# tenstack/batch-scheduler

Measured on NVIDIA H100. Metric: pod_x_node_fit_evals_per_sec, higher is better.
Workload: dtype int64

## Files before the change

### batch-scheduler_b200/csrc/fit.cuh

```cuda
#pragma once
#include "common.cuh"

namespace bsk {

__device__ __forceinline__ uint32_t smem_u32(const void* p) {
  return (uint32_t)__cvta_generic_to_shared(p);
}
__device__ __forceinline__ void mbar_init(uint64_t* bar, uint32_t count) {
  asm volatile("mbarrier.init.shared::cta.b64 [%0], %1;" ::"r"(smem_u32(bar)), "r"(count));
}
__device__ __forceinline__ void mbar_expect_tx(uint64_t* bar, uint32_t bytes) {
  asm volatile("mbarrier.arrive.expect_tx.shared::cta.b64 _, [%0], %1;" ::"r"(smem_u32(bar)), "r"(bytes)
               : "memory");
}
__device__ __forceinline__ void mbar_arrive(uint64_t* bar) {
  asm volatile("mbarrier.arrive.shared::cta.b64 _, [%0];" ::"r"(smem_u32(bar)) : "memory");
}
__device__ __forceinline__ void mbar_wait(uint64_t* bar, uint32_t parity) {
  asm volatile(
      "{\n"
      ".reg .pred p;\n"
      "WAIT_%=:\n"
      "mbarrier.try_wait.parity.shared::cta.b64 p, [%0], %1;\n"
      "@p bra DONE_%=;\n"
// ... 63 lines not shown
  uint32_t* fit_bitmap;
  int64_t* score;
  uint64_t left_w_pitch, left_n_pitch;
  uint64_t score_pitch;
  uint32_t bitmap_pitch;
  uint32_t P, N, Npad, W;
  uint32_t n_full, tail_split;
  unsigned long long* best_packed;
  int32_t* topk_node;
  int64_t* topk_score;
  uint32_t topk_k;
};

template <bool NARROW> struct BestT { using type = int64_t; };
template <> struct BestT<true> { using type = int32_t; };

enum { FIT_OUT_NONE = 0, FIT_OUT_BITMAP = 1, FIT_OUT_SCORE = 2, FIT_OUT_TOPK = 3 };

template <typename S>
__device__ __forceinline__ S topk_insert(S* __restrict__ ls_p, int32_t* __restrict__ ln_p, uint32_t K, uint32_t cb,
                                         S s, int32_t n0 , uint32_t lane) {
  S ls = ls_p[lane];
  int32_t ln = ln_p[lane];
#pragma unroll 1
  do {
    const uint32_t src = __ffs(cb) - 1;
    cb &= cb - 1;
    const S cs = __shfl_sync(0xffffffffu, s, src);
    const int32_t cn = n0 + (int32_t)src;
    const uint32_t pos = __popc(__ballot_sync(0xffffffffu, ls > cs || (ls == cs && ln < cn)));
    if (pos < K) {
      const S us = __shfl_up_sync(0xffffffffu, ls, 1);
      const int32_t un = __shfl_up_sync(0xffffffffu, ln, 1);
      if (lane == pos) { ls = cs; ln = cn; }
      else if (lane > pos) { ls = us; ln = un; }
    }
  } while (cb);
  ls_p[lane] = ls;
  ln_p[lane] = ln;
  return __shfl_sync(0xffffffffu, ls, K - 1);
}

template <int LW, int LN, int LS, int OUT, int RN>
__device__ __forceinline__ void fit_tile(const FitArgs& a, const int64_t* __restrict__ tlw,
                                         const int32_t* __restrict__ tln,
                                         const int64_t (&rqw)[PODS_PER_WARP][LW > 0 ? LW : 1],
                                         const int32_t (&rqn)[PODS_PER_WARP][LN + LS > 0 ? LN + LS : 1],
                                         const ColBits (&colbits)[PODS_PER_WARP], int R0, uint32_t slab ,
                                         uint32_t* s_words, uint32_t wbase , uint32_t node_base, uint32_t lane,
                                         typename BestT<(LN > 0)>::type (&best_s)[PODS_PER_WARP],
                                         int32_t (&best_n)[PODS_PER_WARP], int32_t (&kb)[PODS_PER_WARP],
                                         uint32_t (&cnt)[PODS_PER_WARP],
                                         typename BestT<(LN > 0)>::type* tks, int32_t* tkn ,
                                         typename BestT<(LN > 0)>::type (&thr)[PODS_PER_WARP]) {
  constexpr bool SCORE = OUT == FIT_OUT_SCORE;
  constexpr bool TOPK = OUT == FIT_OUT_TOPK;
  constexpr bool WORDS = OUT == FIT_OUT_BITMAP || SCORE;
  using S = typename BestT<(LN > 0)>::type;
  static_assert(!SCORE || RN == 1, "a staging slab holds one matrix row");
  const int64_t* tpw = tlw + lane;
  const int32_t* tpn = tln + lane;
  int32_t node = (int32_t)(node_base + lane);
  uint32_t wp = smem_u32(s_words) + wbase * 4;
  uint32_t sp = slab + lane * 8;
  int32_t jrem = TILE_WORDS - 1;
#pragma unroll 1
  for (int jb = 0; jb < TILE_WORDS; jb += 4) {
#pragma unroll
    for (int jj = 0; jj < 4; ++jj) {
      int64_t lfw[LW > 0 ? LW : 1];
      int32_t lfn[LN + LS > 0 ? LN + LS : 1];
#pragma unroll
      for (int d = 0; d < LW; ++d) lfw[d] = tpw[d * NODE_TILE + jj * 32];
#pragma unroll
      for (int d = 0; d < LN + LS; ++d) lfn[d] = tpn[d * NODE_TILE + jj * 32];
#pragma unroll
      for (int i = 0; i < RN; ++i) {
        const int r = R0 + i;
        if (LN > 0) {
          int32_t t = lfn[0] - rqn[r][0];
#pragma unroll
          for (int d = 1; d < LN; ++d) t = min(t, lfn[d] - rqn[r][d]);
          uint32_t m32 = (uint32_t)t;
          int32_t sgn = t;
#pragma unroll
          for (int d = 0; d < LS; ++d) {
            const int32_t x = min(lfn[LN + d] - rqn[r][LN + d], (int32_t)a.lm.sclamp[d]);
            sgn |= x;
            m32 = min(m32, (uint32_t)x << a.lm.sshift[d]);
          }
#pragma unroll
          for (int d = 0; d < LW; ++d) {
            const int64_t w = lfw[d] - rqw[r][d];
            const int32_t whi = hi32(w);
            sgn |= whi;
            m32 = min(m32, whi != 0 ? 0xffffffffu : lo32(w));
          }
          const bool fit = (sgn >= 0) && ((colbits[r] >> (jb + jj)) & 1u);
          if (WORDS) sts_u32(wp + (r * 32 + jj) * 4, __ballot_sync(0xffffffffu, fit));
          else if (fit) ++cnt[r];
          if (TOPK && a.fit_bitmap) sts_u32(wp + (r * 32 + jj) * 4, __ballot_sync(0xffffffffu, fit));
          const int32_t key = (int32_t)(m32 << KEY_BITS) + (jrem - jj);
          if (!TOPK && fit) kb[r] = max(kb[r], key);
          if (SCORE) sts_v2u32(sp + jj * 32 * 8, fit ? m32 : 0u, fit ? 0u : 0x80000000u);
          if (TOPK) {
            const uint32_t cb = __ballot_sync(0xffffffffu, fit && (int32_t)m32 > thr[r]);
            if (cb) thr[r] = topk_insert<S>(tks + r * 32, tkn + r * 32, a.topk_k, cb, (int32_t)m32, node + jj * 32 - (int32_t)lane, lane);
          }
        } else {
          int64_t m = lfw[0] - rqw[r][0];
#pragma unroll
          for (int d = 1; d < LW; ++d) m = min64(m, lfw[d] - rqw[r][d]);
          const bool fit = (hi32(m) >= 0) && ((colbits[r] >> (jb + jj)) & 1u);
          if (WORDS) sts_u32(wp + (r * 32 + jj) * 4, __ballot_sync(0xffffffffu, fit));
          else if (fit) ++cnt[r];
          if (TOPK && a.fit_bitmap) sts_u32(wp + (r * 32 + jj) * 4, __ballot_sync(0xffffffffu, fit));
          if (!TOPK && fit && m > best_s[r]) { best_s[r] = m; best_n[r] = node + jj * 32; }
          if (SCORE) sts_u64(sp + jj * 32 * 8, fit ? (long long)m : (long long)INT64_MIN);
          if (TOPK) {
            const uint32_t cb = __ballot_sync(0xffffffffu, fit && m > thr[r]);
            if (cb) thr[r] = topk_insert<S>(tks + r * 32, tkn + r * 32, a.topk_k, cb, m, node + jj * 32 - (int32_t)lane, lane);
          }
        }
      }
    }
    tpw += 128;
    tpn += 128;
    node += 128;
    jrem -= 4;
    wp += 16;
    sp += 128 * 8;
  }
}

__host__ __device__ constexpr size_t fit_tile_bytes(int LW, int LN, int LS) {
  return (size_t)NODE_TILE * (8 * LW + 4 * (LN + LS));
}
__host__ __device__ constexpr size_t fit_slab_bytes() { return (size_t)NODE_TILE * 8; }
__host__ __device__ constexpr size_t fit_topk_bytes() { return (size_t)PODS_PER_CTA * BS_TOPK_MAX * 12; }
static_assert(BS_TOPK_MAX == 32, "a top-K list holds one entry per lane");
__host__ __device__ constexpr size_t fit_smem_front(int LW, int LN, int LS) {
  size_t b = FIT_STAGES * fit_tile_bytes(LW, LN, LS) + (size_t)PODS_PER_CTA * (8 * LW + 4 * (LN + LS));
  b = (b + 7) & ~(size_t)7;
  b += 2 * FIT_STAGES * sizeof(uint64_t) + (size_t)PODS_PER_CTA * 32 * sizeof(uint32_t);
  return (b + 127) & ~(size_t)127;
}
__host__ __device__ constexpr size_t fit_smem_total(int LW, int LN, int LS, int out) {
  return fit_smem_front(LW, LN, LS) + (out == FIT_OUT_SCORE  ? (size_t)FIT_WARPS * FIT_NB * fit_slab_bytes()
                                       : out == FIT_OUT_TOPK ? fit_topk_bytes()
                                                             : 0);
}
constexpr size_t FIT_SMEM_MAX = 227 * 1024;

template <int LW, int LN, int LS, int OUT>
__global__ void __launch_bounds__(FIT_THREADS, FIT_MIN_BLOCKS) gang_fit_kernel(FitArgs a) {
  constexpr bool SCORE = OUT == FIT_OUT_SCORE;
  constexpr bool TOPK = OUT == FIT_OUT_TOPK;
  constexpr bool WORDS = OUT == FIT_OUT_BITMAP || SCORE;
  extern __shared__ __align__(128) unsigned char smem_raw[];
  constexpr size_t STAGE_BYTES = fit_tile_bytes(LW, LN, LS);
  constexpr int LNS = LN + LS;
  unsigned char* s_tile = smem_raw;
  int64_t* s_req_w = reinterpret_cast<int64_t*>(smem_raw + FIT_STAGES * STAGE_BYTES);
  int32_t* s_req_n = reinterpret_cast<int32_t*>(s_req_w + PODS_PER_CTA * LW);
  uint64_t* s_bar = reinterpret_cast<uint64_t*>(
      (reinterpret_cast<uintptr_t>(s_req_n + PODS_PER_CTA * LNS) + 7) & ~(uintptr_t)7);
  uint64_t* s_full = s_bar;
  uint64_t* s_empty = s_bar + FIT_STAGES;
  uint32_t* s_words_all = reinterpret_cast<uint32_t*>(s_bar + 2 * FIT_STAGES);

  const uint32_t tid = threadIdx.x, lane = tid & 31, wid = tid >> 5;
  uint32_t* s_words = s_words_all + wid * PODS_PER_WARP * 32;
  uint32_t unit = blockIdx.x, piece = 0, npieces = 1;
  if (blockIdx.x >= a.n_full) {
    const uint32_t tl = blockIdx.x - a.n_full;
    unit = a.n_full + tl / a.tail_split;
    piece = tl % a.tail_split;
    npieces = a.tail_split;
  }
  const uint32_t pod0 = unit * PODS_PER_CTA;
  const uint32_t wpod0 = pod0 + wid * PODS_PER_WARP;
  const uint32_t n_tiles = a.Npad / NODE_TILE;
  const uint32_t n_lines = (n_tiles + TILES_PER_LINE - 1) / TILES_PER_LINE;
  const uint32_t tile_lo = min(n_tiles, (n_lines * piece / npieces) * TILES_PER_LINE);
  const uint32_t tile_hi = min(n_tiles, (n_lines * (piece + 1) / npieces) * TILES_PER_LINE);

  if (tid == 0) {
    for (int st = 0; st < FIT_STAGES; ++st) {
      mbar_init(&s_full[st], 1);
      mbar_init(&s_empty[st], FIT_WARPS);
    }
    asm volatile("fence.mbarrier_init.release.cluster;" ::: "memory");
  }
  for (uint32_t i = tid; i < PODS_PER_CTA * (LW + LNS); i += FIT_THREADS) {
    const uint32_t pl = i / (LW + LNS), k = i % (LW + LNS);
    const uint32_t p = pod0 + pl;
    const bool is_w = k < (uint32_t)LW;
    const uint32_t kn = k - LW;
    const uint32_t d = is_w ? a.lm.wide[k] : (kn < (uint32_t)LN ? a.lm.narrow[kn] : a.lm.scaled[kn - LN]);
    int64_t v = 0;
    bool present = true;
    if (p < a.P) {
      present = d < 4 || ((a.req_present[p] >> d) & 1u);
      v = present ? a.req[(size_t)d * a.P + p] : 0;
    }
    if (is_w) s_req_w[pl * LW + k] = present ? v : UNCHECKED_REQ;
    else if (kn < (uint32_t)LN) s_req_n[pl * LNS + kn] = present ? (int32_t)v : UNCHECKED_REQ32;
    else s_req_n[pl * LNS + kn] = present ? (int32_t)(v >> a.lm.sunit[kn - LN]) : UNCHECKED_REQS;
  }
  __syncthreads();
  auto issue = [&](uint32_t tile, uint32_t stage) {
    mbar_expect_tx(&s_full[stage], (uint32_t)STAGE_BYTES);
    unsigned char* dst = s_tile + stage * STAGE_BYTES;
    const unsigned char* src_w = reinterpret_cast<const unsigned char*>(a.left_w) + (uint64_t)tile * (NODE_TILE * 8);
    const unsigned char* src_n = reinterpret_cast<const unsigned char*>(a.left_n) + (uint64_t)tile * (NODE_TILE * 4);
#pragma unroll
    for (int d = 0; d < LW; ++d)
      tma_bulk_g2s(dst + (size_t)d * NODE_TILE * 8, src_w + (uint64_t)d * a.left_w_pitch, NODE_TILE * 8,
                   &s_full[stage]);
#pragma unroll
    for (int d = 0; d < LNS; ++d)
      tma_bulk_g2s(dst + (size_t)LW * NODE_TILE * 8 + (size_t)d * NODE_TILE * 4,
                   src_n + (uint64_t)d * a.left_n_pitch, NODE_TILE * 4, &s_full[stage]);
  };
  if (wid == FIT_WARPS) {
    if (lane == 0) {
      if constexpr (SCORE) {
        const uint32_t range = tile_hi - tile_lo;
        for (uint32_t i = 0; i < PODS_PER_WARP * range; ++i) {
          const uint32_t st = i % FIT_STAGES, use = i / FIT_STAGES;
          if (use > 0) mbar_wait(&s_empty[st], (use - 1) & 1);
          issue(tile_lo + i % range, st);
        }
      } else {
        for (uint32_t tile = tile_lo; tile < tile_hi; ++tile) {
          const uint32_t st = (tile - tile_lo) % FIT_STAGES, use = (tile - tile_lo) / FIT_STAGES;
          if (use > 0) mbar_wait(&s_empty[st], (use - 1) & 1);
          issue(tile, st);
        }
      }
    }
    return;
  }

  const bool want_bitmap = a.fit_bitmap != nullptr;
  uint32_t cnt[PODS_PER_WARP];
  typename BestT<(LN > 0)>::type best_s[PODS_PER_WARP];
  int32_t best_n[PODS_PER_WARP];
  int32_t kb[PODS_PER_WARP], kthr[PODS_PER_WARP];
  typename BestT<(LN > 0)>::type thr[PODS_PER_WARP];
  int64_t rqw[PODS_PER_WARP][LW > 0 ? LW : 1];
  int32_t rqn[PODS_PER_WARP][LNS > 0 ? LNS : 1];
  uint32_t coff[PODS_PER_WARP];
  auto load_req = [&](int r) {
#pragma unroll
    for (int d = 0; d < LW; ++d) rqw[r][d] = s_req_w[(wid * PODS_PER_WARP + r) * LW + d];
#pragma unroll
    for (int d = 0; d < LNS; ++d) rqn[r][d] = s_req_n[(wid * PODS_PER_WARP + r) * LNS + d];
  };
  typename BestT<(LN > 0)>::type* tks =
      reinterpret_cast<typename BestT<(LN > 0)>::type*>(smem_raw + fit_smem_front(LW, LN, LS)) + wid * PODS_PER_WARP * 32;
  int32_t* tkn = reinterpret_cast<int32_t*>(smem_raw + fit_smem_front(LW, LN, LS) + (size_t)PODS_PER_CTA * 32 * 8) +
                 wid * PODS_PER_WARP * 32;
#pragma unroll
  for (int r = 0; r < PODS_PER_WARP; ++r) {
    cnt[r] = 0; best_n[r] = -1; kb[r] = -1; kthr[r] = 0; thr[r] = -1;
    if (TOPK) { tks[r * 32 + lane] = -1; tkn[r * 32 + lane] = -1; }
    best_s[r] = LN > 0 ? (typename BestT<(LN > 0)>::type)(-1) : (typename BestT<(LN > 0)>::type)INT64_MIN;
    const uint32_t p = wpod0 + r;
    coff[r] = (p < a.P ? a.fit_class[p] : 0u) * n_tiles * 32 + lane;
    if (!SCORE) load_req(r);
  }
  const uint32_t slab0 = smem_u32(smem_raw + fit_smem_front(LW, LN, LS)) + wid * (uint32_t)(FIT_NB * fit_slab_bytes());
  int64_t* srow = SCORE ? a.score + (size_t)wpod0 * a.score_pitch : nullptr;

  uint32_t stage = 0, phase = 0;
  constexpr int PASSES = SCORE ? PODS_PER_WARP : 1;
  uint32_t nseg = 0, nline = 0;
  ColBits colnext[PODS_PER_WARP];
#pragma unroll
  for (int pass = 0; pass < PASSES; ++pass) {
  if (SCORE) load_req(pass);
#pragma unroll
  for (int r = 0; r < PODS_PER_WARP; ++r)
    if (!SCORE || r == pass) colnext[r] = __ldg(a.classfit + coff[r] + min(tile_lo, n_tiles - 1) * 32);
  for (uint32_t tile = tile_lo; tile < tile_hi; ++tile) {
    ColBits colbits[PODS_PER_WARP];
    const uint32_t tnext = tile + 1 < tile_hi ? tile + 1 : tile;
#pragma unroll
    for (int r = 0; r < PODS_PER_WARP; ++r) {
      if (SCORE && r != pass) continue;
      colbits[r] = colnext[r];
      colnext[r] = __ldg(a.classfit + coff[r] + tnext * 32);
    }
    mbar_wait(&s_full[stage], phase);
    const int64_t* tlw = reinterpret_cast<const int64_t*>(s_tile + stage * STAGE_BYTES);
    const int32_t* tln = reinterpret_cast<const int32_t*>(s_tile + stage * STAGE_BYTES + (size_t)LW * NODE_TILE * 8);
    const uint32_t node_base = tile * NODE_TILE;
    const uint32_t wbase = (tile % TILES_PER_LINE) * TILE_WORDS;
    if constexpr (SCORE) {
      static_assert(PODS_PER_WARP >= FIT_NB, "a bitmap line's word row must be read before it is rewritten");
      const uint32_t wrow = nline % PODS_PER_WARP;
      const uint32_t slab = slab0 + (nseg % FIT_NB) * (uint32_t)fit_slab_bytes();
      if (nseg >= (uint32_t)FIT_NB) {
        if (lane == 0) bulk_wait_read<FIT_NB - 1>();
        __syncwarp();
      }
      fit_tile<LW, LN, LS, OUT, 1>(a, tlw, tln, rqw, rqn, colbits, pass, slab, s_words + ((int)wrow - pass) * 32, wbase,
                                   node_base, lane, best_s, best_n, kb, cnt, tks, tkn, thr);
      fence_async_smem();
      __syncwarp();
      if (lane == 0) {
        if (node_base < (uint32_t)a.score_pitch) {
          const uint32_t cols = min((uint32_t)NODE_TILE, (uint32_t)a.score_pitch - node_base);
          tma_bulk_s2g(srow + (size_t)pass * a.score_pitch + node_base, slab, cols * 8, l2_evict_first());
        }
        if (want_bitmap && ((tile + 1) % TILES_PER_LINE == 0 || tile + 1 == tile_hi))
          tma_bulk_s2g(a.fit_bitmap + (size_t)(wpod0 + pass) * a.bitmap_pitch + (tile / TILES_PER_LINE) * 32,
                       smem_u32(s_words + wrow * 32), (tile % TILES_PER_LINE + 1) * TILE_WORDS * 4, l2_evict_first());
        bulk_commit();
      }
      ++nseg;
    } else {
      fit_tile<LW, LN, LS, OUT, PODS_PER_WARP>(a, tlw, tln, rqw, rqn, colbits, 0, 0, s_words, wbase, node_base, lane,
                                               best_s, best_n, kb, cnt, tks, tkn, thr);
    }
    if (LN > 0 && !TOPK) {
#pragma unroll
      for (int r = 0; r < PODS_PER_WARP; ++r) {
        if (SCORE && r != pass) continue;
        if (kb[r] >= kthr[r]) {
          best_s[r] = kb[r] >> KEY_BITS;
          best_n[r] = (int32_t)(node_base + lane) + (TILE_WORDS - 1 - (kb[r] & (TILE_WORDS - 1))) * 32;
          kthr[r] = (best_s[r] + 1) << KEY_BITS;
        }
        kb[r] = -1;
      }
    }
    __syncwarp();
    if (lane == 0) mbar_arrive(&s_empty[stage]);
    if ((WORDS || (TOPK && want_bitmap)) && ((tile + 1) % TILES_PER_LINE == 0 || tile + 1 == tile_hi)) {
      const uint32_t line = tile / TILES_PER_LINE;
      const uint32_t valid = (tile % TILES_PER_LINE + 1) * TILE_WORDS;
      if constexpr (SCORE) {
        if (lane < valid) cnt[pass] += __popc(s_words[(nline % PODS_PER_WARP) * 32 + lane]);
        ++nline;
      } else if (lane < valid) {
#pragma unroll
        for (int r = 0; r < PODS_PER_WARP; ++r) {
          const uint32_t w = s_words[r * 32 + lane];
          if (WORDS) cnt[r] += __popc(w);
          if (want_bitmap) a.fit_bitmap[(size_t)(wpod0 + r) * a.bitmap_pitch + line * 32 + lane] = w;
        }
      }
    }
    __syncwarp();
    if (++stage == FIT_STAGES) { stage = 0; phase ^= 1; }
  }
  }
  if (SCORE && lane == 0) bulk_wait_read<0>();
  if (TOPK && lane < a.topk_k) {
#pragma unroll
    for (int r = 0; r < PODS_PER_WARP; ++r) {
      const size_t o = (size_t)(wpod0 + r) * a.topk_k + lane;
      const int32_t n = tkn[r * 32 + lane];
      a.topk_node[o] = n;
      a.topk_score[o] = n < 0 ? INT64_MIN : (int64_t)tks[r * 32 + lane];
    }
  }

#pragma unroll
  for (int k = 0; k < PODS_PER_WARP; ++k) {
    int32_t n = TOPK ? tkn[k * 32] : best_n[k];
    int64_t s = n < 0 ? INT64_MIN : TOPK ? (int64_t)tks[k * 32] : (int64_t)best_s[k];
    uint32_t c = cnt[k];
    for (int o = 16; o; o >>= 1) {
      const int64_t os = __shfl_xor_sync(0xffffffffu, s, o);
      const int32_t on = __shfl_xor_sync(0xffffffffu, n, o);
      c += __shfl_xor_sync(0xffffffffu, c, o);
      if (on >= 0 && (n < 0 || os > s || (os == s && on < n))) { s = os; n = on; }
    }
    const uint32_t p = wpod0 + k;
    if (p < a.P && lane == 0) {
      if (npieces == 1) {
        a.feasible_count[p] = c;
        a.best_node[p] = n;
        a.best_score[p] = s;
      } else {
        if (c) atomicAdd(&a.feasible_count[p], c);
        if (n >= 0) atomicMax(&a.best_packed[p], ((unsigned long long)(uint32_t)(s + 1) << 32) | (uint32_t)(~(uint32_t)n));
      }
    }
  }
}

static __global__ void fit_unpack_kernel(const unsigned long long* __restrict__ packed, uint32_t p0, uint32_t P,
                                         int32_t* __restrict__ best_node, int64_t* __restrict__ best_score) {
  const uint32_t p = p0 + blockIdx.x * blockDim.x + threadIdx.x;
  if (p >= P) return;
  const unsigned long long v = packed[p];
  if (v == 0) { best_node[p] = -1; best_score[p] = INT64_MIN; return; }
  best_node[p] = (int32_t)(~(uint32_t)v);
  best_score[p] = (int64_t)(v >> 32) - 1;
}
constexpr uint32_t FIT_TAIL_SPLIT = 8;

}

namespace bsk {
using FitFn = cudaError_t (*)(const FitArgs&, uint32_t units, cudaStream_t, uint32_t* launches, cudaEvent_t ev_a, cudaEvent_t ev_b);
constexpr int FIT_MAX_LN = 8;
constexpr int FIT_N_SLICES = FIT_MAX_LN + 1;
struct FitWS { int lw, ls; };
constexpr FitWS FIT_WS_COMBOS[] = {{0, 0}, {1, 0}, {2, 0}, {3, 0}, {4, 0}, {0, 1}, {0, 2}, {0, 3}, {1, 1}, {1, 2}, {2, 1}};
constexpr int FIT_N_WS = sizeof(FIT_WS_COMBOS) / sizeof(FIT_WS_COMBOS[0]);
inline bool fit_variant_exists(uint32_t LW, uint32_t LN, uint32_t LS) {
  if (LN == 0) return LS == 0 && LW >= 4 && LW <= BS_MAX_LANES;
  if (LN > (uint32_t)FIT_MAX_LN || LW + LN + LS < 4 || LW + LN + LS > BS_MAX_LANES) return false;
  for (int i = 0; i < FIT_N_WS; ++i)
    if ((uint32_t)FIT_WS_COMBOS[i].lw == LW && (uint32_t)FIT_WS_COMBOS[i].ls == LS) return true;
  return false;
}
FitFn fit_lookup_slice0(uint32_t LW, uint32_t LN, uint32_t LS, int out);
FitFn fit_lookup_slice1(uint32_t LW, uint32_t LN, uint32_t LS, int out);
FitFn fit_lookup_slice2(uint32_t LW, uint32_t LN, uint32_t LS, int out);
FitFn fit_lookup_slice3(uint32_t LW, uint32_t LN, uint32_t LS, int out);
FitFn fit_lookup_slice4(uint32_t LW, uint32_t LN, uint32_t LS, int out);
FitFn fit_lookup_slice5(uint32_t LW, uint32_t LN, uint32_t LS, int out);
FitFn fit_lookup_slice6(uint32_t LW, uint32_t LN, uint32_t LS, int out);
FitFn fit_lookup_slice7(uint32_t LW, uint32_t LN, uint32_t LS, int out);
FitFn fit_lookup_slice8(uint32_t LW, uint32_t LN, uint32_t LS, int out);
inline FitFn fit_lookup(uint32_t LW, uint32_t LN, uint32_t LS, int out) {
  switch (LN) {
    case 0: return fit_lookup_slice0(LW, LN, LS, out);
    case 1: return fit_lookup_slice1(LW, LN, LS, out);
    case 2: return fit_lookup_slice2(LW, LN, LS, out);
    case 3: return fit_lookup_slice3(LW, LN, LS, out);
    case 4: return fit_lookup_slice4(LW, LN, LS, out);
    case 5: return fit_lookup_slice5(LW, LN, LS, out);
    case 6: return fit_lookup_slice6(LW, LN, LS, out);
    case 7: return fit_lookup_slice7(LW, LN, LS, out);
    case 8: return fit_lookup_slice8(LW, LN, LS, out);
  }
  return nullptr;
}
}
```

### batch-scheduler_b200/csrc/fit_inst.cu

```cuda
#include <algorithm>

#include "fit.cuh"

#ifndef BS_FIT_SLICE
#error "compile with -DBS_FIT_SLICE=<0..8>"
#endif

namespace bsk {
namespace {

template <int LW, int LN, int LS, int OUT>
cudaError_t launch_fit_t(const FitArgs& a0, uint32_t units, cudaStream_t s, uint32_t* launches, cudaEvent_t ev_a, cudaEvent_t ev_b) {
  constexpr size_t smem = fit_smem_total(LW, LN, LS, OUT);
  static_assert(smem <= FIT_SMEM_MAX, "the fit kernel's shared memory exceeds what one CTA may use");
  cudaError_t er = cudaFuncSetAttribute(gang_fit_kernel<LW, LN, LS, OUT>, cudaFuncAttributeMaxDynamicSharedMemorySize,
                                        (int)smem);
  if (er != cudaSuccess) return er;
  FitArgs a = a0;
  a.n_full = units;
  a.tail_split = 1;
  if (LN > 0 && OUT != FIT_OUT_TOPK && a.best_packed && units) {
    int per_sm = 0, dev = 0, sms = 0;
    if (cudaOccupancyMaxActiveBlocksPerMultiprocessor(&per_sm, gang_fit_kernel<LW, LN, LS, OUT>, FIT_THREADS, smem) == cudaSuccess &&
        cudaGetDevice(&dev) == cudaSuccess && cudaDeviceGetAttribute(&sms, cudaDevAttrMultiProcessorCount, dev) == cudaSuccess &&
        per_sm > 0 && sms > 0) {
      const uint32_t slots = (uint32_t)per_sm * (uint32_t)sms;
      const uint32_t n_tiles = a.Npad / NODE_TILE, n_lines = (n_tiles + TILES_PER_LINE - 1) / TILES_PER_LINE;
      const uint32_t n_full = units / slots * slots, tail = units - n_full;
      const uint32_t split = std::min<uint32_t>(FIT_TAIL_SPLIT, n_lines);
      if (tail && split > 1 && tail * 10 < slots * 9) {
        a.n_full = n_full;
        a.tail_split = split;
      }
    }
  }
  const uint32_t tail_units = units - a.n_full;
  if (a.tail_split > 1) {
    const uint32_t p0 = a.n_full * PODS_PER_CTA;
    if (p0 < a.P) {
      er = cudaMemsetAsync(a.feasible_count + p0, 0, (size_t)(a.P - p0) * 4, s);
      if (er == cudaSuccess) er = cudaMemsetAsync(a.best_packed + p0, 0, (size_t)(a.P - p0) * 8, s);
      if (er != cudaSuccess) return er;
    }
  }
  if (ev_a) cudaEventRecord(ev_a, s);
  gang_fit_kernel<LW, LN, LS, OUT><<<a.n_full + tail_units * a.tail_split, FIT_THREADS, smem, s>>>(a);
  if (ev_b) cudaEventRecord(ev_b, s);
  if (launches) *launches = 1;
  if (a.tail_split > 1) {
    const uint32_t p0 = a.n_full * PODS_PER_CTA;
    if (p0 < a.P) {
      fit_unpack_kernel<<<(a.P - p0 + 255) / 256, 256, 0, s>>>(a.best_packed, p0, a.P, a.best_node, a.best_score);
      if (launches) *launches = 2;
    }
  }
  return cudaGetLastError();
}

template <int LW, int LN, int LS>
FitFn pick(int out) {
  switch (out) {
    case FIT_OUT_SCORE: return launch_fit_t<LW, LN, LS, FIT_OUT_SCORE>;
    case FIT_OUT_BITMAP: return launch_fit_t<LW, LN, LS, FIT_OUT_BITMAP>;
    case FIT_OUT_TOPK: return launch_fit_t<LW, LN, LS, FIT_OUT_TOPK>;
  }
  return launch_fit_t<LW, LN, LS, FIT_OUT_NONE>;
}

}

#define BS_CAT2(a, b) a##b
#define BS_CAT(a, b) BS_CAT2(a, b)

FitFn BS_CAT(fit_lookup_slice, BS_FIT_SLICE)(uint32_t LW, uint32_t LN, uint32_t LS, int score) {
#if BS_FIT_SLICE == 0
  if (LN != 0 || LS != 0) return nullptr;
  switch (LW) {
    case 4: return pick<4, 0, 0>(score);
    case 6: return pick<6, 0, 0>(score);
    case 7: return pick<7, 0, 0>(score);
    case 8: return pick<8, 0, 0>(score);
    case 9: return pick<9, 0, 0>(score);
    case 10: return pick<10, 0, 0>(score);
    case 11: return pick<11, 0, 0>(score);
    case 12: return pick<12, 0, 0>(score);
    case 13: return pick<13, 0, 0>(score);
    case 14: return pick<14, 0, 0>(score);
    case 15: return pick<15, 0, 0>(score);
    case 16: return pick<16, 0, 0>(score);
    case 5: return pick<5, 0, 0>(score);
  }
  return nullptr;
#else
  constexpr int N = BS_FIT_SLICE;
  if (LN != (uint32_t)N || !fit_variant_exists(LW, LN, LS)) return nullptr;
  const uint32_t key = LW * 8 + LS;
  switch (key) {
#define BS_CASE(lw, ls)                                                        \
  case lw * 8 + ls:                                                            \
    if constexpr (lw + N + ls >= 4) return pick<lw, N, ls>(score); else break;
    BS_CASE(0, 0) BS_CASE(1, 0) BS_CASE(2, 0) BS_CASE(3, 0) BS_CASE(4, 0) BS_CASE(0, 1) BS_CASE(0, 2) BS_CASE(0, 3)
    BS_CASE(1, 1) BS_CASE(1, 2) BS_CASE(2, 1)
#undef BS_CASE
  }
  return nullptr;
#endif
}

}
```

### profiles/microbench/store_ladder.cu

```cuda
#include <algorithm>
#include <cstdint>
#include <cstdio>
#include <cstdlib>
#include <vector>
#include <cuda_runtime.h>

namespace {

constexpr int T = 512;
constexpr int NB = 2;
constexpr int LANES = 5;
constexpr uint32_t STAGE = LANES * T * 4;
constexpr uint32_t SLAB = T * 8;
constexpr int PODS_PER_CTA = 32;
constexpr uint32_t P = 100000, N = 10000;

__device__ __forceinline__ uint32_t smem_u32(const void* p) { return (uint32_t)__cvta_generic_to_shared(p); }
__device__ __forceinline__ void mbar_init(uint64_t* bar, uint32_t count) {
  asm volatile("mbarrier.init.shared::cta.b64 [%0], %1;" ::"r"(smem_u32(bar)), "r"(count));
}
__device__ __forceinline__ void mbar_expect_tx(uint64_t* bar, uint32_t bytes) {
  asm volatile("mbarrier.arrive.expect_tx.shared::cta.b64 _, [%0], %1;" ::"r"(smem_u32(bar)), "r"(bytes) : "memory");
}
__device__ __forceinline__ void mbar_arrive(uint64_t* bar) {
// ... 29 lines not shown
struct LArgs {
  long long* out;
  uint32_t* bitmap;
  const int32_t* left;
  uint32_t* cnt;
  unsigned long long* packed;
  int32_t* best;
  uint32_t Npad, pitch, bitmap_pitch, n_full, tail_split;
};

__host__ __device__ constexpr uint32_t front_bytes(int stages, int bm) {
  uint32_t b = stages * STAGE + PODS_PER_CTA * LANES * 4;
  b = (b + 7) & ~7u;
  b += 2 * stages * 8 + (bm == 2 ? 2 : 1) * PODS_PER_CTA * 32 * 4;
  return (b + 127) & ~127u;
}
__host__ __device__ constexpr uint32_t smem_bytes(int stages, int bm) { return front_bytes(stages, bm) + 8 * NB * SLAB; }

template <bool HINT, bool RING, int RPW, int BM, bool SPLIT, int STAGES, bool PAIR, bool FB = false>
__global__ void __launch_bounds__(288, 2) ladder(LArgs a) {
  static_assert(!PAIR || STAGES >= 3, "a pod's tile pair and the next tile's load need three stages");
  static_assert(!FB || (RING && !PAIR), "front to back: one row per pass over the ring's tiles");
  constexpr int PASSES = FB ? RPW : 1, ROWS = FB ? 1 : RPW;
  extern __shared__ __align__(128) unsigned char smem[];
  constexpr uint32_t FRONT = front_bytes(STAGES, BM);
  uint64_t* full = reinterpret_cast<uint64_t*>(smem + ((STAGES * STAGE + PODS_PER_CTA * LANES * 4 + 7) & ~7u));
  uint64_t* empty = full + STAGES;
  uint32_t* words_all = reinterpret_cast<uint32_t*>(empty + STAGES);
  const uint32_t tid = threadIdx.x, lane = tid & 31, wid = tid >> 5;
  uint32_t unit = blockIdx.x, piece = 0, npieces = 1;
  if (SPLIT && blockIdx.x >= a.n_full) {
    const uint32_t tl = blockIdx.x - a.n_full;
    unit = a.n_full + tl / a.tail_split;
    piece = tl % a.tail_split;
    npieces = a.tail_split;
  }
  const uint32_t row0 = unit * (8 * RPW) + wid * RPW;
  const uint32_t n_tiles = a.Npad / T, n_lines = (n_tiles + 1) / 2;
  const uint32_t tile_lo = min(n_tiles, (n_lines * piece / npieces) * 2);
  const uint32_t tile_hi = min(n_tiles, (n_lines * (piece + 1) / npieces) * 2);
  if (RING) {
    if (tid == 0) {
      for (int s = 0; s < STAGES; ++s) {
        mbar_init(&full[s], 1);
        mbar_init(&empty[s], 8);
      }
      asm volatile("fence.mbarrier_init.release.cluster;" ::: "memory");
    }
    __syncthreads();
    if (wid == 8) {
      if (lane == 0)
        for (uint32_t i = 0; i < PASSES * (tile_hi - tile_lo); ++i) {
          const uint32_t t = tile_lo + i % (tile_hi - tile_lo), st = i % STAGES, use = i / STAGES;
          if (use > 0) mbar_wait(&empty[st], (use - 1) & 1);
          mbar_expect_tx(&full[st], STAGE);
          for (int d = 0; d < LANES; ++d)
            g2s(smem + st * STAGE + d * T * 4, a.left + (size_t)d * a.Npad + (size_t)t * T, T * 4, &full[st]);
        }
      return;
    }
  } else if (wid >= 8) {
    return;
  }
  const uint32_t slab0 = smem_u32(smem + FRONT) + wid * NB * SLAB;
  uint32_t* words = words_all + wid * RPW * 32;
  uint32_t stage = 0, phase = 0, sb = 0, nseg = 0, bmbuf = 0;
  constexpr uint32_t STEP = PAIR ? 2 : 1;
  for (int pass = 0; pass < PASSES; ++pass)
  for (uint32_t tile = tile_lo; tile < tile_hi; tile += STEP) {
    const uint32_t nt = min(STEP, tile_hi - tile);
    if (RING) {
      uint32_t s = stage, ph = phase;
      for (uint32_t k = 0; k < nt; ++k) {
        mbar_wait(&full[s], ph);
        if (++s == STAGES) { s = 0; ph ^= 1; }
      }
    }
#pragma unroll
    for (int rr = 0; rr < ROWS; ++rr) {
      const int r = FB ? pass : rr;
      for (uint32_t k = 0; k < nt; ++k) {
        const uint32_t t = tile + k, node_base = t * T;
        const uint32_t slab = slab0 + sb * SLAB;
        if (nseg >= NB) {
          if (lane == 0) bulk_wait_read1();
          __syncwarp();
        }
#pragma unroll 4
        for (int j = 0; j < T / 32; ++j)
          asm volatile("st.shared.u64 [%0], %1;" ::"r"(slab + (j * 32 + lane) * 8), "l"((long long)(node_base + j * 32 + lane)));
        if (BM && lane < T / 32) words[(BM == 2 ? bmbuf * PODS_PER_CTA * 32 : 0) + r * 32 + (t & 1) * (T / 32) + lane] = 0xffffffffu;
        fence_async_smem();
        __syncwarp();
        if (lane == 0) {
          if (node_base < a.pitch)
            s2g<HINT>(a.out + (size_t)(row0 + r) * a.pitch + node_base, slab, min((uint32_t)T, a.pitch - node_base) * 8);
          bulk_commit();
        }
        ++nseg;
        sb ^= 1;
      }
    }
    if (RING) {
      __syncwarp();
      for (uint32_t k = 0; k < nt; ++k) {
        if (lane == 0) mbar_arrive(&empty[stage]);
        if (++stage == STAGES) { stage = 0; phase ^= 1; }
      }
    }
    const uint32_t tlast = tile + nt - 1;
    if (BM && ((tlast + 1) % 2 == 0 || tlast + 1 == tile_hi)) {
      const uint32_t line = tlast / 2, valid = (tlast % 2 + 1) * (T / 32);
      __syncwarp();
      if (BM == 1) {
        if (lane < valid)
#pragma unroll
          for (int rr = 0; rr < ROWS; ++rr) {
            const int r = FB ? pass : rr;
            a.bitmap[(size_t)(row0 + r) * a.bitmap_pitch + line * 32 + lane] = words[r * 32 + lane];
          }
      } else {
        fence_async_smem();
        __syncwarp();
        if (lane == 0)
#pragma unroll
          for (int rr = 0; rr < ROWS; ++rr) {
            const int r = FB ? pass : rr;
            s2g<true>(a.bitmap + (size_t)(row0 + r) * a.bitmap_pitch + line * 32,
                      smem_u32(words + bmbuf * PODS_PER_CTA * 32 + r * 32), valid * 4);
          }
        bmbuf ^= 1;
      }
    }
  }
  if (lane == 0) {
    if (BM == 2) bulk_commit();
    bulk_wait_read0();
  }
  if (SPLIT && lane == 0) {
#pragma unroll
    for (int r = 0; r < RPW; ++r) {
      const uint32_t p = row0 + r;
      if (npieces == 1) {
        a.cnt[p] = tile_hi - tile_lo;
        a.best[p] = (int32_t)p;
      } else {
        atomicAdd(&a.cnt[p], tile_hi - tile_lo);
        atomicMax(&a.packed[p], ((unsigned long long)(piece + 1) << 32) | p);
      }
    }
  }
}

struct Rung {
  const char* name;
  void (*fn)(LArgs);
  bool ring, split;
  int rpw;
  uint32_t smem;
};
template <bool HINT, bool RING, int RPW, int BM, bool SPLIT, int STAGES, bool PAIR, bool FB = false>
Rung rung(const char* name) {
  return {name, ladder<HINT, RING, RPW, BM, SPLIT, STAGES, PAIR, FB>, RING, SPLIT, RPW, smem_bytes(STAGES, BM)};
}

#define CK(x)                                                                            \
  do {                                                                                   \
    cudaError_t e_ = (x);                                                                \
    if (e_ != cudaSuccess) {                                                             \
      fprintf(stderr, "%s:%d %s: %s\n", __FILE__, __LINE__, #x, cudaGetErrorString(e_)); \
      exit(1);                                                                           \
    }                                                                                    \
  } while (0)

}

int main(int argc, char** argv) {
  const int rounds = argc > 1 ? atoi(argv[1]) : 3;
  const int iters = argc > 2 ? atoi(argv[2]) : 25;
  const char* power = argc > 3 ? argv[3] : "unknown";
  const int round0 = argc > 4 ? atoi(argv[4]) : 0;
  const uint32_t Npad = (N + T - 1) / T * T, pitch = N, bitmap_pitch = ((N + 31) / 32 + 31) & ~31u;
  LArgs a{};
  CK(cudaMalloc(&a.out, (size_t)P * pitch * 8));
  CK(cudaMalloc(&a.bitmap, (size_t)P * bitmap_pitch * 4));
  CK(cudaMalloc(&a.left, (size_t)LANES * Npad * 4));
  CK(cudaMemset((void*)a.left, 0, (size_t)LANES * Npad * 4));
  CK(cudaMalloc(&a.cnt, P * 4));
  CK(cudaMalloc(&a.packed, P * 8));
  CK(cudaMalloc(&a.best, P * 4));
  a.Npad = Npad;
  a.pitch = pitch;
  a.bitmap_pitch = bitmap_pitch;
  cudaDeviceProp prop;
  CK(cudaGetDeviceProperties(&prop, 0));

  const std::vector<Rung> rungs = {
      rung<false, false, 1, 0, false, 2, false>("r0_base"),
      rung<true, false, 1, 0, false, 2, false>("r1_hint"),
      rung<true, true, 1, 0, false, 2, false>("r2_ring"),
      rung<true, true, 4, 0, false, 2, false>("r3_rows4"),
      rung<true, true, 4, 1, false, 2, false>("r4_bitmap"),
      rung<true, true, 4, 1, true, 2, false>("r5_grid"),
      rung<true, true, 4, 1, true, 3, false>("r5_stages3"),
      rung<true, true, 4, 1, true, 3, true>("r5_pair"),
      rung<true, true, 4, 2, true, 2, false>("r5_bmbulk"),
      rung<true, true, 1, 0, false, 3, false>("r2_stages3"),
      rung<true, true, 4, 0, false, 2, false, true>("r3_fb"),
      rung<true, true, 2, 0, false, 2, false>("r3_rows2"),
      rung<true, true, 4, 2, true, 2, false, true>("r5_bmbulk_fb"),
  };
  cudaEvent_t e0, e1;
  CK(cudaEventCreate(&e0));
  CK(cudaEventCreate(&e1));
  for (int rd = 0; rd < rounds; ++rd) {
    for (const Rung& g : rungs) {
      const uint32_t smem = std::max<uint32_t>(g.smem, smem_bytes(2, 1));
      CK(cudaFuncSetAttribute(g.fn, cudaFuncAttributeMaxDynamicSharedMemorySize, (int)smem));
      const int threads = g.ring ? 288 : 256;
      int occ = 0;
      CK(cudaOccupancyMaxActiveBlocksPerMultiprocessor(&occ, g.fn, threads, smem));
      const uint32_t units = P / (8 * g.rpw);
      LArgs b = a;
      b.n_full = units;
      b.tail_split = 1;
      if (g.split) {
        const uint32_t slots = (uint32_t)occ * prop.multiProcessorCount, n_lines = (Npad / T + 1) / 2;
        const uint32_t n_full = units / slots * slots, tail = units - n_full, split = std::min<uint32_t>(8, n_lines);
        if (tail && split > 1 && tail * 10 < slots * 9) {
          b.n_full = n_full;
          b.tail_split = split;
        }
      }
      const uint32_t grid = b.n_full + (units - b.n_full) * b.tail_split;
      auto launch = [&] {
        if (g.split && b.tail_split > 1) {
          const uint32_t p0 = b.n_full * PODS_PER_CTA;
          CK(cudaMemsetAsync(b.cnt + p0, 0, (size_t)(P - p0) * 4));
          CK(cudaMemsetAsync(b.packed + p0, 0, (size_t)(P - p0) * 8));
        }
        CK(cudaEventRecord(e0));
        g.fn<<<grid, threads, smem>>>(b);
        CK(cudaEventRecord(e1));
        CK(cudaEventSynchronize(e1));
      };
      CK(cudaMemset(a.out, 0xff, (size_t)P * pitch * 8));
      for (int i = 0; i < 3; ++i) launch();
      std::vector<float> ms(iters);
      for (int i = 0; i < iters; ++i) {
        launch();
        CK(cudaEventElapsedTime(&ms[i], e0, e1));
      }
      CK(cudaGetLastError());
      std::sort(ms.begin(), ms.end());
      bool ok = true;
      for (uint32_t row : {0u, P / 2 + 7, P - 1})
        for (uint32_t n : {0u, 511u, N - 1}) {
          long long v;
          CK(cudaMemcpy(&v, a.out + (size_t)row * pitch + n, 8, cudaMemcpyDeviceToHost));
          ok = ok && v == (long long)n;
        }
      printf("{\"rung\": \"%s\", \"round\": %d, \"median_ms\": %.4f, \"min_ms\": %.4f, \"iters\": %d, \"grid\": %u, "
             "\"threads\": %d, \"smem\": %u, \"ctas_per_sm\": %d, \"ok\": %s, \"gpu\": \"%s\", \"power_limit_w\": \"%s\"}\n",
             g.name, round0 + rd, ms[iters / 2], ms[0], iters, grid, threads, smem, occ, ok ? "true" : "false", prop.name, power);
      fflush(stdout);
    }
  }
  return 0;
}
```

Baseline: 365.6 billion.

## Add node-block-resident score kernel that keeps a node block in shared memory across pods

Adds a new score-mode kernel for shapes with narrow dimensions. Each CTA loads one line's worth of node tiles into shared memory once with bulk TMA and then sweeps a chunk of pods over it, instead of streaming node tiles through a staged ring for every pod group. When there are several node blocks, partial counts and best nodes are merged with atomics plus an unpack kernel. This adds memsets and a second launch, and it lowers per-CTA pod parallelism. The microbenchmark ladder also gains resident-variant rungs.

```diff
diff --git a/batch-scheduler_b200/csrc/fit.cuh b/batch-scheduler_b200/csrc/fit.cuh
--- a/batch-scheduler_b200/csrc/fit.cuh
+++ b/batch-scheduler_b200/csrc/fit.cuh
@@ -239,8 +239,47 @@
 }
 constexpr size_t FIT_SMEM_MAX = 227 * 1024;
 
+template <int LW, int LN, int LS>
+__device__ __forceinline__ void fit_stage_req(const FitArgs& a, uint32_t p, uint32_t pl, uint32_t k, int64_t* s_req_w,
+                                              int32_t* s_req_n) {
+  constexpr int LNS = LN + LS;
+  const bool is_w = k < (uint32_t)LW;
+  const uint32_t kn = k - LW;
+  const uint32_t d = is_w ? a.lm.wide[k] : (kn < (uint32_t)LN ? a.lm.narrow[kn] : a.lm.scaled[kn - LN]);
+  int64_t v = 0;
+  bool present = true;
+  if (p < a.P) {
+    present = d < 4 || ((a.req_present[p] >> d) & 1u);
+    v = present ? a.req[(size_t)d * a.P + p] : 0;
+  }
+  if (is_w) s_req_w[pl * LW + k] = present ? v : UNCHECKED_REQ;
+  else if (kn < (uint32_t)LN) s_req_n[pl * LNS + kn] = present ? (int32_t)v : UNCHECKED_REQ32;
+  else s_req_n[pl * LNS + kn] = present ? (int32_t)(v >> a.lm.sunit[kn - LN]) : UNCHECKED_REQS;
+}
+
+__device__ __forceinline__ void fit_pod_result(const FitArgs& a, uint32_t p, uint32_t c, int64_t s, int32_t n,
+                                               bool whole, uint32_t lane) {
+  for (int o = 16; o; o >>= 1) {
+    const int64_t os = __shfl_xor_sync(0xffffffffu, s, o);
+    const int32_t on = __shfl_xor_sync(0xffffffffu, n, o);
+    c += __shfl_xor_sync(0xffffffffu, c, o);
+    if (on >= 0 && (n < 0 || os > s || (os == s && on < n))) { s = os; n = on; }
+  }
+  if (p < a.P && lane == 0) {
+    if (whole) {
+      a.feasible_count[p] = c;
+      a.best_node[p] = n;
+      a.best_score[p] = s;
+    } else {
+      if (c) atomicAdd(&a.feasible_count[p], c);
+      if (n >= 0) atomicMax(&a.best_packed[p], ((unsigned long long)(uint32_t)(s + 1) << 32) | (uint32_t)(~(uint32_t)n));
+    }
+  }
+}
+
 template <int LW, int LN, int LS, int OUT>
 __global__ void __launch_bounds__(FIT_THREADS, FIT_MIN_BLOCKS) gang_fit_kernel(FitArgs a) {
+  static_assert(OUT != FIT_OUT_SCORE || LN == 0, "narrow score shapes run gang_fit_score_kernel");
   constexpr bool SCORE = OUT == FIT_OUT_SCORE;
   constexpr bool TOPK = OUT == FIT_OUT_TOPK;
   constexpr bool WORDS = OUT == FIT_OUT_BITMAP || SCORE;
@@ -415,7 +454,6 @@
     if (LN > 0 && !TOPK) {
 #pragma unroll
       for (int r = 0; r < PODS_PER_WARP; ++r) {
-        if (SCORE && r != pass) continue;
         if (kb[r] >= kthr[r]) {
           best_s[r] = kb[r] >> KEY_BITS;
           best_n[r] = (int32_t)(node_base + lane) + (TILE_WORDS - 1 - (kb[r] & (TILE_WORDS - 1))) * 32;
@@ -479,6 +517,121 @@
       }
     }
   }
+}
+
+constexpr int FIT_SCORE_PPW = 2;
+constexpr int FIT_SCORE_PODS = FIT_WARPS * FIT_SCORE_PPW;
+constexpr int FIT_BLOCK_NODES = TILES_PER_LINE * NODE_TILE;
+constexpr int FIT_SCORE_THREADS = FIT_WARPS * 32;
+__host__ __device__ constexpr size_t fit_score_smem_front(int LW, int LN, int LS) {
+  const size_t b = TILES_PER_LINE * fit_tile_bytes(LW, LN, LS) + FIT_WARPS * 2 * 32 * sizeof(uint32_t) +
+                   sizeof(uint64_t) + (size_t)FIT_SCORE_PODS * (8 * LW + 4 * (LN + LS));
+  return (b + 127) & ~(size_t)127;
+}
+__host__ __device__ constexpr size_t fit_score_smem_total(int LW, int LN, int LS) {
+  return fit_score_smem_front(LW, LN, LS) + (size_t)FIT_WARPS * FIT_NB * fit_slab_bytes();
+}
+
+template <int LW, int LN, int LS>
+__global__ void __launch_bounds__(FIT_SCORE_THREADS, FIT_MIN_BLOCKS) gang_fit_score_kernel(FitArgs a, uint32_t n_blocks) {
+  static_assert(LN > 0, "the all-wide shapes' best key does not fit the packed 32-bit form");
+  static_assert(FIT_NB == TILES_PER_LINE, "a line buffer is rewritten two pods later, behind the slab wait that covers its read");
+  constexpr int LNS = LN + LS;
+  constexpr size_t TILE_BYTES = fit_tile_bytes(LW, LN, LS);
+  using S = int32_t;
+  extern __shared__ __align__(128) unsigned char smem_raw[];
+  uint32_t* s_words_all = reinterpret_cast<uint32_t*>(smem_raw + TILES_PER_LINE * TILE_BYTES);
+  uint64_t* s_bar = reinterpret_cast<uint64_t*>(s_words_all + FIT_WARPS * 2 * 32);
+  int64_t* s_req_w = reinterpret_cast<int64_t*>(s_bar + 1);
+  int32_t* s_req_n = reinterpret_cast<int32_t*>(s_req_w + FIT_SCORE_PODS * LW);
+  const uint32_t tid = threadIdx.x, lane = tid & 31, wid = tid >> 5;
+  const uint32_t blk = blockIdx.x % n_blocks, pod0 = blockIdx.x / n_blocks * FIT_SCORE_PODS;
+  const uint32_t n_tiles = a.Npad / NODE_TILE, tile0 = blk * TILES_PER_LINE;
+  const uint32_t nt = min((uint32_t)TILES_PER_LINE, n_tiles - tile0);
+  if (tid == 0) {
+    mbar_init(s_bar, 1);
+    asm volatile("fence.mbarrier_init.release.cluster;" ::: "memory");
+    mbar_expect_tx(s_bar, nt * (uint32_t)TILE_BYTES);
+    for (uint32_t t = 0; t < nt; ++t) {
+      unsigned char* dst = smem_raw + t * TILE_BYTES;
+      const unsigned char* src_w = reinterpret_cast<const unsigned char*>(a.left_w) + (uint64_t)(tile0 + t) * (NODE_TILE * 8);
+      const unsigned char* src_n = reinterpret_cast<const unsigned char*>(a.left_n) + (uint64_t)(tile0 + t) * (NODE_TILE * 4);
+#pragma unroll
+      for (int d = 0; d < LW; ++d)
+        tma_bulk_g2s(dst + (size_t)d * NODE_TILE * 8, src_w + (uint64_t)d * a.left_w_pitch, NODE_TILE * 8, s_bar);
+#pragma unroll
+      for (int d = 0; d < LNS; ++d)
+        tma_bulk_g2s(dst + (size_t)LW * NODE_TILE * 8 + (size_t)d * NODE_TILE * 4, src_n + (uint64_t)d * a.left_n_pitch,
+                     NODE_TILE * 4, s_bar);
+    }
+  }
+  for (uint32_t i = tid; i < FIT_SCORE_PODS * (LW + LNS); i += FIT_SCORE_THREADS)
+    fit_stage_req<LW, LN, LS>(a, pod0 + i / (LW + LNS), i / (LW + LNS), i % (LW + LNS), s_req_w, s_req_n);
+  auto cls = [&](uint32_t p) { return a.classfit + (size_t)(p < a.P ? a.fit_class[p] : 0u) * n_tiles * 32 + lane; };
+  const ColBits* cls_p = cls(pod0 + wid);
+  ColBits colnext = __ldg(cls_p + tile0 * 32);
+  __syncthreads();
+  mbar_wait(s_bar, 0);
+
+  const bool want_bitmap = a.fit_bitmap != nullptr;
+  const uint32_t slab0 = smem_u32(smem_raw + fit_score_smem_front(LW, LN, LS)) + wid * (uint32_t)(FIT_NB * fit_slab_bytes());
+  uint32_t nseg = 0;
+#pragma unroll 1
+  for (uint32_t k = 0; k < FIT_SCORE_PPW; ++k) {
+    const uint32_t pl = k * FIT_WARPS + wid, p = pod0 + pl;
+    if (p >= a.P) break;
+    int64_t rqw[PODS_PER_WARP][LW > 0 ? LW : 1];
+    int32_t rqn[PODS_PER_WARP][LNS];
+#pragma unroll
+    for (int d = 0; d < LW; ++d) rqw[0][d] = s_req_w[pl * LW + d];
+#pragma unroll
+    for (int d = 0; d < LNS; ++d) rqn[0][d] = s_req_n[pl * LNS + d];
+    uint32_t* s_words = s_words_all + (wid * 2 + (k & 1)) * 32;
+    int64_t* srow = a.score + (size_t)p * a.score_pitch;
+    const ColBits* cls_next = k + 1 < FIT_SCORE_PPW ? cls(p + FIT_WARPS) : cls_p;
+    uint32_t cnt[PODS_PER_WARP] = {0};
+    S best_s[PODS_PER_WARP] = {-1}, thr[PODS_PER_WARP];
+    int32_t best_n[PODS_PER_WARP] = {-1}, kb[PODS_PER_WARP] = {-1}, kthr = 0;
+#pragma unroll 1
+    for (uint32_t t = 0; t < nt; ++t) {
+      ColBits colbits[PODS_PER_WARP];
+      colbits[0] = colnext;
+      colnext = __ldg(t + 1 < nt ? cls_p + (tile0 + t + 1) * 32 : cls_next + tile0 * 32);
+      const uint32_t node_base = (tile0 + t) * NODE_TILE, slab = slab0 + (nseg % FIT_NB) * (uint32_t)fit_slab_bytes();
+      if (nseg >= (uint32_t)FIT_NB) {
+        if (lane == 0) bulk_wait_read<FIT_NB - 1>();
+        __syncwarp();
+      }
+      const unsigned char* tile = smem_raw + t * TILE_BYTES;
+      fit_tile<LW, LN, LS, FIT_OUT_SCORE, 1>(a, reinterpret_cast<const int64_t*>(tile),
+                                             reinterpret_cast<const int32_t*>(tile + (size_t)LW * NODE_TILE * 8), rqw, rqn,
+                                             colbits, 0, slab, s_words, t * TILE_WORDS, node_base, lane, best_s, best_n,
+                                             kb, cnt, (S*)nullptr, nullptr, thr);
+      fence_async_smem();
+      __syncwarp();
+      if (lane == 0) {
+        if (node_base < (uint32_t)a.score_pitch) {
+          const uint32_t cols = min((uint32_t)NODE_TILE, (uint32_t)a.score_pitch - node_base);
+          tma_bulk_s2g(srow + node_base, slab, cols * 8, l2_evict_first());
+        }
+        if (want_bitmap && t + 1 == nt)
+          tma_bulk_s2g(a.fit_bitmap + (size_t)p * a.bitmap_pitch + blk * 32, smem_u32(s_words), nt * TILE_WORDS * 4,
+                       l2_evict_first());
+        bulk_commit();
+      }
+      ++nseg;
+      if (kb[0] >= kthr) {
+        best_s[0] = kb[0] >> KEY_BITS;
+        best_n[0] = (int32_t)(node_base + lane) + (TILE_WORDS - 1 - (kb[0] & (TILE_WORDS - 1))) * 32;
+        kthr = (best_s[0] + 1) << KEY_BITS;
+      }
+      kb[0] = -1;
+    }
+    if (lane < nt * TILE_WORDS) cnt[0] += __popc(s_words[lane]);
+    fit_pod_result(a, p, cnt[0], best_n[0] < 0 ? INT64_MIN : (int64_t)best_s[0], best_n[0], n_blocks == 1, lane);
+    cls_p = cls_next;
+  }
+  if (lane == 0) bulk_wait_read<0>();
 }
 
 static __global__ void fit_unpack_kernel(const unsigned long long* __restrict__ packed, uint32_t p0, uint32_t P,
diff --git a/batch-scheduler_b200/csrc/fit_inst.cu b/batch-scheduler_b200/csrc/fit_inst.cu
--- a/batch-scheduler_b200/csrc/fit_inst.cu
+++ b/batch-scheduler_b200/csrc/fit_inst.cu
@@ -9,8 +9,33 @@
 namespace bsk {
 namespace {
 
+template <int LW, int LN, int LS>
+cudaError_t launch_fit_score(const FitArgs& a, cudaStream_t s, uint32_t* launches, cudaEvent_t ev_a, cudaEvent_t ev_b) {
+  constexpr size_t smem = fit_score_smem_total(LW, LN, LS);
+  static_assert(smem <= FIT_SMEM_MAX, "the fit kernel's shared memory exceeds what one CTA may use");
+  cudaError_t er = cudaFuncSetAttribute(gang_fit_score_kernel<LW, LN, LS>, cudaFuncAttributeMaxDynamicSharedMemorySize,
+                                        (int)smem);
+  if (er != cudaSuccess) return er;
+  const uint32_t n_blocks = (a.Npad + FIT_BLOCK_NODES - 1) / FIT_BLOCK_NODES;
+  const uint32_t n_chunks = (a.P + FIT_SCORE_PODS - 1) / FIT_SCORE_PODS;
+  if (n_blocks > 1) {
+    er = cudaMemsetAsync(a.feasible_count, 0, (size_t)a.P * 4, s);
+    if (er == cudaSuccess) er = cudaMemsetAsync(a.best_packed, 0, (size_t)a.P * 8, s);
+    if (er != cudaSuccess) return er;
+  }
+  if (ev_a) cudaEventRecord(ev_a, s);
+  gang_fit_score_kernel<LW, LN, LS><<<n_blocks * n_chunks, FIT_SCORE_THREADS, smem, s>>>(a, n_blocks);
+  if (ev_b) cudaEventRecord(ev_b, s);
+  if (launches) *launches = 1;
+  if (n_blocks > 1) {
+    fit_unpack_kernel<<<(a.P + 255) / 256, 256, 0, s>>>(a.best_packed, 0, a.P, a.best_node, a.best_score);
+    if (launches) *launches = 2;
+  }
+  return cudaGetLastError();
+}
+
 template <int LW, int LN, int LS, int OUT>
-cudaError_t launch_fit_t(const FitArgs& a0, uint32_t units, cudaStream_t s, uint32_t* launches, cudaEvent_t ev_a, cudaEvent_t ev_b) {
+cudaError_t launch_fit_units(const FitArgs& a0, uint32_t units, cudaStream_t s, uint32_t* launches, cudaEvent_t ev_a, cudaEvent_t ev_b) {
   constexpr size_t smem = fit_smem_total(LW, LN, LS, OUT);
   static_assert(smem <= FIT_SMEM_MAX, "the fit kernel's shared memory exceeds what one CTA may use");
   cudaError_t er = cudaFuncSetAttribute(gang_fit_kernel<LW, LN, LS, OUT>, cudaFuncAttributeMaxDynamicSharedMemorySize,
@@ -55,6 +80,12 @@
     }
   }
   return cudaGetLastError();
+}
+
+template <int LW, int LN, int LS, int OUT>
+cudaError_t launch_fit_t(const FitArgs& a, uint32_t units, cudaStream_t s, uint32_t* launches, cudaEvent_t ev_a, cudaEvent_t ev_b) {
+  if constexpr (OUT == FIT_OUT_SCORE && LN > 0) return launch_fit_score<LW, LN, LS>(a, s, launches, ev_a, ev_b);
+  else return launch_fit_units<LW, LN, LS, OUT>(a, units, s, launches, ev_a, ev_b);
 }
 
 template <int LW, int LN, int LS>
diff --git a/profiles/microbench/store_ladder.cu b/profiles/microbench/store_ladder.cu
--- a/profiles/microbench/store_ladder.cu
+++ b/profiles/microbench/store_ladder.cu
@@ -205,16 +205,81 @@
   }
 }
 
+constexpr int BLK = 1024;
+constexpr uint32_t RES_BLOCK = LANES * BLK * 4;
+constexpr uint32_t RES_LINES = (RES_BLOCK + 8 + 127) & ~127u;
+constexpr uint32_t RES_FRONT = RES_LINES + 8 * 2 * 128;
+constexpr uint32_t RES_SMEM = RES_FRONT + 8 * NB * SLAB;
+static_assert(P % 8 == 0, "every octet of pods is whole");
+
+__global__ void __launch_bounds__(256, 2) resident(LArgs a, uint32_t n_blocks, uint32_t n_chunks) {
+  extern __shared__ __align__(128) unsigned char smem[];
+  uint64_t* bar = reinterpret_cast<uint64_t*>(smem + RES_BLOCK);
+  const uint32_t tid = threadIdx.x, lane = tid & 31, wid = tid >> 5;
+  const uint32_t b = blockIdx.x % n_blocks, c = blockIdx.x / n_blocks;
+  const uint32_t node0 = b * BLK, nodes = min((uint32_t)BLK, a.Npad - node0), n_oct = P / 8;
+  const uint32_t p_lo = n_oct * c / n_chunks * 8, p_hi = n_oct * (c + 1) / n_chunks * 8;
+  if (tid == 0) {
+    mbar_init(bar, 1);
+    asm volatile("fence.mbarrier_init.release.cluster;" ::: "memory");
+    mbar_expect_tx(bar, LANES * nodes * 4);
+    for (int d = 0; d < LANES; ++d) g2s(smem + d * BLK * 4, a.left + (size_t)d * a.Npad + node0, nodes * 4, bar);
+  }
+  __syncthreads();
+  mbar_wait(bar, 0);
+  const uint32_t slab0 = smem_u32(smem + RES_FRONT) + wid * NB * SLAB;
+  uint32_t* lines = reinterpret_cast<uint32_t*>(smem + RES_LINES) + wid * 2 * 32;
+  uint32_t nseg = 0, k = 0;
+  for (uint32_t p = p_lo + wid; p < p_hi; p += 8, ++k) {
+    uint32_t* words = lines + (k & 1) * 32;
+    for (uint32_t h = 0; h * T < nodes; ++h) {
+      const uint32_t node_base = node0 + h * T, slab = slab0 + (nseg & 1) * SLAB;
+      if (nseg >= NB) {
+        if (lane == 0) bulk_wait_read1();
+        __syncwarp();
+      }
+#pragma unroll 4
+      for (int j = 0; j < T / 32; ++j)
+        asm volatile("st.shared.u64 [%0], %1;" ::"r"(slab + (j * 32 + lane) * 8), "l"((long long)(node_base + j * 32 + lane)));
+      if (lane < T / 32) words[h * (T / 32) + lane] = 0xffffffffu;
+      fence_async_smem();
+      __syncwarp();
+      if (lane == 0) {
+        if (node_base < a.pitch)
+          s2g<true>(a.out + (size_t)p * a.pitch + node_base, slab, min((uint32_t)T, a.pitch - node_base) * 8);
+        if ((h + 1) * T >= nodes)
+          s2g<true>(a.bitmap + (size_t)p * a.bitmap_pitch + b * 32, smem_u32(words), nodes / 32 * 4);
+        bulk_commit();
+      }
+      ++nseg;
+    }
+    if (lane == 0) {
+      if (n_blocks == 1) {
+        a.cnt[p] = nodes;
+        a.best[p] = (int32_t)p;
+      } else {
+        atomicAdd(&a.cnt[p], nodes);
+        atomicMax(&a.packed[p], ((unsigned long long)(b + 1) << 32) | p);
+      }
+    }
+  }
+  if (lane == 0) bulk_wait_read0();
+}
+
 struct Rung {
   const char* name;
   void (*fn)(LArgs);
   bool ring, split;
   int rpw;
   uint32_t smem;
+  uint32_t res_mult, res_opc;
 };
 template <bool HINT, bool RING, int RPW, int BM, bool SPLIT, int STAGES, bool PAIR, bool FB = false>
 Rung rung(const char* name) {
-  return {name, ladder<HINT, RING, RPW, BM, SPLIT, STAGES, PAIR, FB>, RING, SPLIT, RPW, smem_bytes(STAGES, BM)};
+  return {name, ladder<HINT, RING, RPW, BM, SPLIT, STAGES, PAIR, FB>, RING, SPLIT, RPW, smem_bytes(STAGES, BM), 0, 0};
+}
+Rung resident_rung(const char* name, uint32_t mult, uint32_t opc = 0) {
+  return {name, nullptr, false, true, 1, RES_SMEM, mult, opc};
 }
 
 #define CK(x)                                                                            \
@@ -262,12 +327,61 @@
       rung<true, true, 4, 0, false, 2, false, true>("r3_fb"),
       rung<true, true, 2, 0, false, 2, false>("r3_rows2"),
       rung<true, true, 4, 2, true, 2, false, true>("r5_bmbulk_fb"),
+      resident_rung("r6_resident", 1),
+      resident_rung("r6_resident_x4", 4),
+      resident_rung("r6_resident_x16", 16),
+      resident_rung("r6_resident_x64", 64),
+      resident_rung("r6_oct1", 0, 1),
+      resident_rung("r6_oct2", 0, 2),
+      resident_rung("r6_oct4", 0, 4),
   };
   cudaEvent_t e0, e1;
   CK(cudaEventCreate(&e0));
   CK(cudaEventCreate(&e1));
+  auto times = [&](const Rung& g, auto&& launch, uint32_t grid, int threads, uint32_t smem, int occ, int rd) {
+    CK(cudaMemset(a.out, 0xff, (size_t)P * pitch * 8));
+    for (int i = 0; i < 3; ++i) launch();
+    std::vector<float> ms(iters);
+    for (int i = 0; i < iters; ++i) {
+      launch();
+      CK(cudaEventElapsedTime(&ms[i], e0, e1));
+    }
+    CK(cudaGetLastError());
+    std::sort(ms.begin(), ms.end());
+    bool ok = true;
+    for (uint32_t row : {0u, P / 2 + 7, P - 1})
+      for (uint32_t n : {0u, 511u, 1024u, N - 1}) {
+        long long v;
+        CK(cudaMemcpy(&v, a.out + (size_t)row * pitch + n, 8, cudaMemcpyDeviceToHost));
+        ok = ok && v == (long long)n;
+      }
+    printf("{\"rung\": \"%s\", \"round\": %d, \"median_ms\": %.4f, \"min_ms\": %.4f, \"iters\": %d, \"grid\": %u, "
+           "\"threads\": %d, \"smem\": %u, \"ctas_per_sm\": %d, \"ok\": %s, \"gpu\": \"%s\", \"power_limit_w\": \"%s\"}\n",
+           g.name, round0 + rd, ms[iters / 2], ms[0], iters, grid, threads, smem, occ, ok ? "true" : "false", prop.name, power);
+    fflush(stdout);
+  };
   for (int rd = 0; rd < rounds; ++rd) {
     for (const Rung& g : rungs) {
+      if (g.res_mult || g.res_opc) {
+        CK(cudaFuncSetAttribute(resident, cudaFuncAttributeMaxDynamicSharedMemorySize, (int)g.smem));
+        int occ = 0;
+        CK(cudaOccupancyMaxActiveBlocksPerMultiprocessor(&occ, resident, 256, g.smem));
+        const uint32_t slots = (uint32_t)occ * prop.multiProcessorCount, n_blocks = (Npad + BLK - 1) / BLK;
+        uint32_t g0 = slots, nb = n_blocks;
+        while (nb) { const uint32_t t = g0 % nb; g0 = nb; nb = t; }
+        const uint32_t n_chunks = g.res_mult ? std::min<uint32_t>(P / 8, slots / g0 * g.res_mult) : (P / 8 + g.res_opc - 1) / g.res_opc;
+        const uint32_t grid = n_blocks * n_chunks;
+        auto launch = [&] {
+          CK(cudaMemsetAsync(a.cnt, 0, (size_t)P * 4));
+          CK(cudaMemsetAsync(a.packed, 0, (size_t)P * 8));
+          CK(cudaEventRecord(e0));
+          resident<<<grid, 256, g.smem>>>(a, n_blocks, n_chunks);
+          CK(cudaEventRecord(e1));
+          CK(cudaEventSynchronize(e1));
+        };
+        times(g, launch, grid, 256, g.smem, occ, rd);
+        continue;
+      }
       const uint32_t smem = std::max<uint32_t>(g.smem, smem_bytes(2, 1));
       CK(cudaFuncSetAttribute(g.fn, cudaFuncAttributeMaxDynamicSharedMemorySize, (int)smem));
       const int threads = g.ring ? 288 : 256;
@@ -297,26 +411,7 @@
         CK(cudaEventRecord(e1));
         CK(cudaEventSynchronize(e1));
       };
-      CK(cudaMemset(a.out, 0xff, (size_t)P * pitch * 8));
-      for (int i = 0; i < 3; ++i) launch();
-      std::vector<float> ms(iters);
-      for (int i = 0; i < iters; ++i) {
-        launch();
-        CK(cudaEventElapsedTime(&ms[i], e0, e1));
-      }
-      CK(cudaGetLastError());
-      std::sort(ms.begin(), ms.end());
-      bool ok = true;
-      for (uint32_t row : {0u, P / 2 + 7, P - 1})
-        for (uint32_t n : {0u, 511u, N - 1}) {
-          long long v;
-          CK(cudaMemcpy(&v, a.out + (size_t)row * pitch + n, 8, cudaMemcpyDeviceToHost));
-          ok = ok && v == (long long)n;
-        }
-      printf("{\"rung\": \"%s\", \"round\": %d, \"median_ms\": %.4f, \"min_ms\": %.4f, \"iters\": %d, \"grid\": %u, "
-             "\"threads\": %d, \"smem\": %u, \"ctas_per_sm\": %d, \"ok\": %s, \"gpu\": \"%s\", \"power_limit_w\": \"%s\"}\n",
-             g.name, round0 + rd, ms[iters / 2], ms[0], iters, grid, threads, smem, occ, ok ? "true" : "false", prop.name, power);
-      fflush(stdout);
+      times(g, launch, grid, threads, smem, occ, rd);
     }
   }
   return 0;
```

Measured after the change: 369.4 billion (median of 6 runs). +1.0%, better.
